# vimalmanohar/old-kaldi-git

Measured on AMD Instinct MI355X. Metric: frames/sec decoded + real-time factor, LibriSpeech nnet2 decode @1/2/4/8 MI355X, higher is better.
Workload: dtype f32

## Files before the change

### old-kaldi-git_amd/csrc/kh_decoder.hip

```cpp
#include <algorithm>
#include <cstddef>
#include <cstdint>

#include "kh_common.h"
#include "kh_decoder_types.h"

using namespace kh;
using namespace kh::dec;

namespace {

__device__ __forceinline__ unsigned KhOpaqueTidX() {
  unsigned t = threadIdx.x;
  asm volatile("" : "+v"(t));
  return t;
}
#define KH_TIDX (KhOpaqueTidX())

#ifdef KH_SERVE_MARKERS
__device__ int32_t *g_serve_mark = nullptr;
#define KM(k, aux) do { if (KH_TIDX == 0 && g_serve_mark != nullptr) __hip_atomic_store(g_serve_mark + blockIdx.x * 16 + 13, ((k) << 24) | (static_cast<int32_t>(aux) & 0xffffff), __ATOMIC_RELAXED, __HIP_MEMORY_SCOPE_SYSTEM); } while (0)
__device__ int32_t *g_wave_mark = nullptr;
#define WM(k, aux) do { if ((KH_TIDX & 63) == 0 && g_wave_mark != nullptr) __hip_atomic_store(g_wave_mark + blockIdx.x * 64 + (KH_TIDX >> 6), ((k) << 24) | (static_cast<int32_t>(aux) & 0xffffff), __ATOMIC_RELAXED, __HIP_MEMORY_SCOPE_SYSTEM); } while (0)
#define WM_ANY(c) (__any(c) ? (1 << 20) : 0)
// ... 1892 lines not shown
      if (cnt != n_new) sh->status = cnt < 0 ? 3 : 8;
    }
  }
  KhSync();
  SubStamp(u, sh, 50);
  if (Uni(sh->status) != 0) return false;
  for (int i = ne_emit + KH_TIDX; i < fe; i += NT)
    __hip_atomic_fetch_min(&UX(x_bmin)[UX(x_bkt)[i - nb]], UX(x_q)[i - nb], __ATOMIC_RELAXED, __HIP_MEMORY_SCOPE_AGENT);
  KhSync();
  {
    constexpr int kOU = 4;
    for (int i0 = KH_TIDX; i0 < n; i0 += NT * kOU) {
      int32_t bk[kOU];
      uint32_t qv[kOU], bm[kOU];
#pragma unroll
      for (int k = 0; k < kOU; k++) {
        const int i = min(i0 + k * NT, n - 1);
        bk[k] = UX(x_bkt)[i];
        qv[k] = UX(x_q)[i];
      }
#pragma unroll
      for (int k = 0; k < kOU; k++) bm[k] = __hip_atomic_load(&UX(x_bmin)[bk[k]], __ATOMIC_RELAXED, __HIP_MEMORY_SCOPE_AGENT);
#pragma unroll
      for (int k = 0; k < kOU; k++) {
        const int i = i0 + k * NT;
        if (i >= n) continue;
        UX(x_key0)[i] = (static_cast<unsigned long long>(bm[k]) << 32) | qv[k];
        UX(x_val0)[i] = i;
      }
    }
  }
  KhSync();
  {
    constexpr int kOU = 4;
    for (int i0 = KH_TIDX; i0 < n; i0 += NT * kOU) {
      int32_t bk[kOU];
#pragma unroll
      for (int k = 0; k < kOU; k++) bk[k] = UX(x_bkt)[min(i0 + k * NT, n - 1)];
#pragma unroll
      for (int k = 0; k < kOU; k++)
        if (i0 + k * NT < n) UX(x_bmin)[bk[k]] = 0xFFFFFFFFu;
    }
  }
  const int fb2 = n > 1 ? BlockRadixSort(u, n, bits, sh) : 0;
  KhSync();
  const Arr<const int32_t> order = fb2 ? UX(x_val1) : UX(x_val0);
  {
    constexpr int kOU = 8;
    for (int r0 = KH_TIDX; r0 < n; r0 += NT * kOU) {
      int32_t o[kOU];
#pragma unroll
      for (int k = 0; k < kOU; k++) o[k] = order[min(r0 + k * NT, n - 1)];
#pragma unroll
      for (int k = 0; k < kOU; k++)
        if (r0 + k * NT < n) UX(x_pos)[o[k]] = r0 + k * NT;
    }
  }
  KhSync();
  SubStamp(u, sh, 51);
  return true;
}

constexpr int kFastN = 65535, kFastNew = 1024, kFastMulti = 2 * kLdsSlots;

__device__ __forceinline__ int OpaqueTid() {
  int t = static_cast<int>(threadIdx.x);
  asm volatile("" : "+v"(t));
  return t;
}
struct TidRef {
  __device__ __forceinline__ operator int() const { return OpaqueTid(); }
};

__device__ __forceinline__ int BitmapPrefix(LdsU32 bits, LdsU32 pre, int W, Blk &sh) {
  const TidRef tid;
  constexpr int kPer = kLdsSlots / NT;
  int c[kPer], mine = 0;
#pragma unroll
  for (int j = 0; j < kPer; j++) {
    const int w = tid * kPer + j;
    const uint32_t v = bits[w];
    c[j] = w < W ? __popc(v) : 0;
    mine += c[j];
  }
  int total;
  int run = BlockExScan<true>(mine, &total, sh);
#pragma unroll
  for (int j = 0; j < kPer; j++) {
    const int w = tid * kPer + j;
    if (w < W) pre[w] = static_cast<uint32_t>(run);
    run += c[j];
  }
  return total;
}
__device__ __forceinline__ int LdsExScanInPlace(LdsU32 a, int W, Blk &sh) {
  const TidRef tid;
  constexpr int kPer = kLdsSlots / NT;
  int c[kPer], mine = 0;
#pragma unroll
  for (int j = 0; j < kPer; j++) {
    const int w = tid * kPer + j;
    const uint32_t v = a[w];
    c[j] = w < W ? static_cast<int>(v) : 0;
    mine += c[j];
  }
  int total;
  int run = BlockExScan<true>(mine, &total, sh);
#pragma unroll
  for (int j = 0; j < kPer; j++) {
    const int w = tid * kPer + j;
    if (w < W) a[w] = static_cast<uint32_t>(run);
    run += c[j];
  }
  return total;
}
__device__ __forceinline__ int BitRank(LdsU32 bits, LdsU32 pre, uint32_t q) {
  return static_cast<int>(pre[q >> 5]) + __popc(bits[q >> 5] & ((1u << (q & 31u)) - 1u));
}

__device__ void ReplayFromMemory(const Utt &u, const Params &p, int nb, int fe, int lb, int le, float cutoff, uint32_t qbase, Blk &sh) {
  const int ne_emit = Uni(sh->x_ne_emit), eps_emit = Uni(sh->x_eps_emit), eps_n = Uni(sh->eps_n), n_new = fe - ne_emit;
  for (int j = KH_TIDX; j < eps_n; j += NT) {
    const int tok = u.tmp_epslist[j];
    UX(x_epsidx)[tok - nb] = j;
    UX(x_nl0)[j] = 0;
    UX(x_nl1)[j] = 0;
    UX(x_ncost)[j] = j < eps_emit ? Dec(UX(x_c0e)[j]) : INFINITY;
  }
  for (int i = ne_emit + KH_TIDX; i < fe; i += NT) UX(x_q)[i - nb] = 0xFFFFFFFFu;
  KhSync();
  for (int l = lb + KH_TIDX; l < le; l += NT) {
    const int src = u.link_src[l], dst = u.link_dst[l];
    const int j = UX(x_epsidx)[src - nb];
    if (l == lb || u.link_src[l - 1] != src) UX(x_nl0)[j] = l - lb;
    if (l + 1 == le || u.link_src[l + 1] != src) UX(x_nl1)[j] = l - lb + 1;
    int code = -1;
    if (dst >= 0) {
      const int e = UX(x_epsidx)[dst - nb];
      if (e >= 0) code = e;
      else if (dst >= ne_emit) code = 0x40000000 | (dst - nb);
    }
    UX(x_ord)[l - lb] = code;
    UX(x_lw)[l - lb] = __int_as_float(p.n_arcs[-1 - u.link_arc[l]].z);
  }
  KhSync();
  if (KH_TIDX == 0) {
    const int cnt = ReplayClosure((GP(float))UX(x_ncost).p, (GP(int32_t))UX(x_nl0).p, (GP(int32_t))UX(x_nl1).p, (GP(int32_t))UX(x_ord).p,
                                  (GP(float))UX(x_lw).p, (GP(int32_t))UX(x_stack).p, 0, u, sh, eps_emit, cutoff, nb, qbase, n_new);
    if (cnt != n_new) sh->status = cnt < 0 ? 3 : 8;
  }
  KhSync();
}

__device__ void PositionsFromHeads(const Utt &u, int cnt, Blk &sh, int xs0) {
  const TidRef tid;
  const LdsU32 K = (LdsU32)LdsKeys(sh);
  constexpr int kU = 8;
  int pbase = 0;
  for (int h0 = 0; h0 < cnt; h0 += kLdsSlots) {
    const uint32_t W = static_cast<uint32_t>(min(kLdsSlots, cnt - h0));
    for (uint32_t w = tid; w < W; w += NT) K[w] = 0u;
    LdsSync();
    XS(xs0 + 0);
    for (int i0 = tid; i0 < cnt; i0 += NT * kU) {
      int hh[kU];
#pragma unroll
      for (int k = 0; k < kU; k++) hh[k] = UX(x_h)[min(i0 + k * NT, cnt - 1)];
#pragma unroll
      for (int k = 0; k < kU; k++) {
        const uint32_t at = static_cast<uint32_t>(hh[k] - h0);
        if (i0 + k * NT < cnt && at < W) (void)__hip_atomic_fetch_add(&K[at], 1u, __ATOMIC_RELAXED, __HIP_MEMORY_SCOPE_WORKGROUP);
      }
    }
    LdsSync();
    XS(xs0 + 1);
    const int total = LdsExScanInPlace(K, static_cast<int>(W), sh);
    LdsSync();
    XS(xs0 + 2);
    for (int i0 = tid; i0 < cnt; i0 += NT * kU) {
      int hh[kU], ib[kU];
#pragma unroll
      for (int k = 0; k < kU; k++) {
        const int i = min(i0 + k * NT, cnt - 1);
        hh[k] = UX(x_h)[i];
        ib[k] = UX(x_inb)[i];
      }
#pragma unroll
      for (int k = 0; k < kU; k++) {
        const uint32_t at = static_cast<uint32_t>(hh[k] - h0);
        if (i0 + k * NT < cnt && at < W) UX(x_pos)[i0 + k * NT] = pbase + static_cast<int>(K[at]) + ib[k];
      }
    }
    pbase += total;
    LdsSync();
    XS(xs0 + 3);
  }
}

__device__ int OrderFrontierFast(const Utt &u, const Params &p, int nb, int fe, int lb, int le, float cutoff, Blk &sh) {
  const TidRef tid;
  const int ne_emit = Uni(sh->x_ne_emit), n = fe - nb, n_emit = ne_emit - nb, eps_emit = Uni(sh->x_eps_emit), eps_n = Uni(sh->eps_n);
  const uint32_t H = Uni(sh->x_hsize), qbase = Uni(sh->x_qbase);
  const int nl = le - lb, n_new = fe - ne_emit;
  const LdsU32 K = (LdsU32)LdsKeys(sh), V = (LdsU32)LdsVals(sh);
  const LdsU16 V16 = (LdsU16)LdsVals(sh);
  const int Hw = static_cast<int>((H + 31u) >> 5), qw = static_cast<int>((qbase + 31u) >> 5);
  const Arr<int32_t> xr = UX(x_val0);
  constexpr int kU = 8;
  if (u.phase_cycles != nullptr && tid == 0) {
    sh->t_sub = static_cast<long long>(__builtin_amdgcn_s_memtime());
    sh->phase[47] += 1; sh->phase[52] += eps_emit; sh->phase[53] += eps_n; sh->phase[54] += nl; sh->phase[55] += n_new; sh->phase[46] += n;
  }
  const bool comb = qw + 2 * Hw <= kLdsSlots;
  const int o1 = comb ? qw : 0, o2 = o1 + Hw, W1 = o2 + Hw;
  if (!comb) {
    int rbase = 0;
    for (uint32_t c0 = 0; c0 < qbase; c0 += static_cast<uint32_t>(kLdsSlots) * 32u) {
      const int W = min(kLdsSlots, static_cast<int>((qbase - c0 + 31u) >> 5));
      for (int w = tid; w < W; w += NT) K[w] = 0u;
      LdsSync();
      XS(0);
      for (int i = tid; i < n_emit; i += NT) {
        const uint32_t q = UX(x_q)[i] - c0;
        if (q < static_cast<uint32_t>(kLdsSlots) * 32u) (void)__hip_atomic_fetch_or(&K[q >> 5], 1u << (q & 31u), __ATOMIC_RELAXED, __HIP_MEMORY_SCOPE_WORKGROUP);
      }
      LdsSync();
      XS(1);
      const int total = BitmapPrefix(K, V, W, sh);
      LdsSync();
      XS(2);
      for (int i = tid; i < n_emit; i += NT) {
        const uint32_t q = UX(x_q)[i] - c0;
        if (q < static_cast<uint32_t>(kLdsSlots) * 32u) xr[i] = rbase + BitRank(K, V, q);
      }
      rbase += total;
      LdsSync();
      XS(3);
    }
  }
  for (int w = tid; w < W1; w += NT) K[w] = 0u;
  LdsSync();
  XS(4);
  for (int i0 = tid; i0 < n; i0 += NT * kU) {
    int32_t sid[kU];
    uint32_t qv[kU];
#pragma unroll
    for (int k = 0; k < kU; k++) {
      const int i = min(i0 + k * NT, n - 1);
      sid[k] = i < n_emit ? UX(x_bkt)[i] : -1 - p.unit_ilabel[u.tok_state[nb + i]];
      qv[k] = UX(x_q)[i];
    }
#pragma unroll
    for (int k = 0; k < kU; k++) {
      const int i = i0 + k * NT;
      if (i >= n) continue;
      const uint32_t bk = static_cast<uint32_t>(sid[k]) % H;
      UX(x_bkt)[i] = static_cast<int32_t>(bk);
      UX(x_epsidx)[i] = -1;
      if (i < n_emit) {
        const uint32_t m = 1u << (bk & 31u);
        const uint32_t old = __hip_atomic_fetch_or(&K[o1 + (bk >> 5)], m, __ATOMIC_RELAXED, __HIP_MEMORY_SCOPE_WORKGROUP);
        if ((old & m) != 0u) (void)__hip_atomic_fetch_or(&K[o2 + (bk >> 5)], m, __ATOMIC_RELAXED, __HIP_MEMORY_SCOPE_WORKGROUP);
        if (comb) (void)__hip_atomic_fetch_or(&K[qv[k] >> 5], 1u << (qv[k] & 31u), __ATOMIC_RELAXED, __HIP_MEMORY_SCOPE_WORKGROUP);
      }
    }
  }
  LdsSync();
  XS(5);
  for (int i = n_emit + static_cast<int>((tid + NT - n_emit % NT) % NT); i < n; i += NT) {
    const uint32_t bk = static_cast<uint32_t>(UX(x_bkt)[i]), m = 1u << (bk & 31u);
    if ((K[o1 + (bk >> 5)] & m) != 0u) (void)__hip_atomic_fetch_or(&K[o2 + (bk >> 5)], m, __ATOMIC_RELAXED, __HIP_MEMORY_SCOPE_WORKGROUP);
  }
  LdsSync();
  XS(6);
  const int n_bits = BitmapPrefix(K, V, W1, sh);
  LdsSync();
  XS(7);
  const int pre2 = static_cast<int>(V[o2]);
  const int n_b2 = n_bits - pre2;
  if (n_b2 > kLdsSlots) return 2;
  for (int i0 = tid; i0 < n; i0 += NT * kU) {
    uint32_t bks[kU], qv[kU];
#pragma unroll
    for (int k = 0; k < kU; k++) {
      const int i = min(i0 + k * NT, n - 1);
      bks[k] = static_cast<uint32_t>(UX(x_bkt)[i]);
      qv[k] = (comb || i >= n_emit) ? UX(x_q)[i] : static_cast<uint32_t>(xr[i]);
    }
#pragma unroll
    for (int k = 0; k < kU; k++) {
      const int i = i0 + k * NT;
      if (i >= n) continue;
      const uint32_t bk = bks[k], m = 1u << (bk & 31u);
      const int w2 = o2 + static_cast<int>(bk >> 5);
      const uint32_t bits2 = K[w2];
      const int r = i < n_emit ? (comb ? BitRank(K, V, qv[k]) : static_cast<int>(qv[k])) : -1;
      if (comb && i < n_emit) xr[i] = r;
      if ((bits2 & m) != 0u) {
        UX(x_bkt)[i] = static_cast<int>(V[w2]) - pre2 + __popc(bits2 & (m - 1u));
      } else {
        UX(x_bkt)[i] = i < n_emit ? -1 : -2 - static_cast<int32_t>(bk);
        UX(x_h)[i] = r;
        UX(x_inb)[i] = 0;
      }
    }
  }
// ... 303 lines not shown
  const int o1 = comb ? qw : 0, o2 = o1 + Hw, W1 = o2 + Hw;
  const LdsU32 P = comb ? K + W1 : K + qw;
  const LdsU32 P2 = comb ? K + W1 + o2 : K + 2 * Hw;
  if (tid == 0) sh->flag = 0;
  if (!comb) {
    for (int w = tid; w < qw; w += NT) K[w] = 0u;
    LdsSync();
    for (int i0 = tid; i0 < n; i0 += NT * kU) {
      int32_t sid[kU];
      uint32_t qv[kU];
#pragma unroll
      for (int k = 0; k < kU; k++) {
        const int i = min(i0 + k * NT, n - 1);
        sid[k] = i < n_emit ? UX(x_bkt)[i] : -1 - p.unit_ilabel[u.tok_state[nb + i]];
        qv[k] = UX(x_q)[i];
      }
#pragma unroll
      for (int k = 0; k < kU; k++) {
        const int i = i0 + k * NT;
        if (i >= n) continue;
        T[i] = static_cast<uint32_t>(sid[k]) % H;
        if (i < n_emit) (void)__hip_atomic_fetch_or(&K[qv[k] >> 5], 1u << (qv[k] & 31u), __ATOMIC_RELAXED, __HIP_MEMORY_SCOPE_WORKGROUP);
      }
    }
    LdsSync();
    (void)BitmapPrefix(K, P, qw, sh);
    LdsSync();
    for (int i = tid; i < n_emit; i += NT) T[i] |= static_cast<uint32_t>(BitRank(K, P, UX(x_q)[i])) << 17;
    LdsSync();
    for (int w = tid; w < 2 * Hw; w += NT) K[w] = 0u;
    LdsSync();
    for (int i = tid; i < n_emit; i += NT) {
      const uint32_t bk = T[i] & 0x1ffffu, m = 1u << (bk & 31u);
      const uint32_t old = __hip_atomic_fetch_or(&K[o1 + (bk >> 5)], m, __ATOMIC_RELAXED, __HIP_MEMORY_SCOPE_WORKGROUP);
      if ((old & m) != 0u) (void)__hip_atomic_fetch_or(&K[o2 + (bk >> 5)], m, __ATOMIC_RELAXED, __HIP_MEMORY_SCOPE_WORKGROUP);
    }
  } else {
    for (int w = tid; w < W1; w += NT) K[w] = 0u;
    LdsSync();
    for (int i0 = tid; i0 < n; i0 += NT * kU) {
      int32_t sid[kU];
      uint32_t qv[kU];
#pragma unroll
      for (int k = 0; k < kU; k++) {
        const int i = min(i0 + k * NT, n - 1);
        sid[k] = i < n_emit ? UX(x_bkt)[i] : -1 - p.unit_ilabel[u.tok_state[nb + i]];
        qv[k] = UX(x_q)[i];
      }
#pragma unroll
      for (int k = 0; k < kU; k++) {
        const int i = i0 + k * NT;
        if (i >= n) continue;
        const uint32_t bk = static_cast<uint32_t>(sid[k]) % H;
        T[i] = bk;
        if (i < n_emit) {
          const uint32_t m = 1u << (bk & 31u);
          const uint32_t old = __hip_atomic_fetch_or(&K[o1 + (bk >> 5)], m, __ATOMIC_RELAXED, __HIP_MEMORY_SCOPE_WORKGROUP);
          if ((old & m) != 0u) (void)__hip_atomic_fetch_or(&K[o2 + (bk >> 5)], m, __ATOMIC_RELAXED, __HIP_MEMORY_SCOPE_WORKGROUP);
          (void)__hip_atomic_fetch_or(&K[qv[k] >> 5], 1u << (qv[k] & 31u), __ATOMIC_RELAXED, __HIP_MEMORY_SCOPE_WORKGROUP);
        }
      }
    }
  }
  LdsSync();
  for (int i = n_emit + tid; i < n; i += NT) {
    const uint32_t bk = T[i] & 0x1ffffu, m = 1u << (bk & 31u);
    if ((K[o1 + (bk >> 5)] & m) != 0u) (void)__hip_atomic_fetch_or(&K[o2 + (bk >> 5)], m, __ATOMIC_RELAXED, __HIP_MEMORY_SCOPE_WORKGROUP);
  }
  LdsSync();
  int n_b2;
  uint32_t pre2 = 0u;
  if (comb) {
    const int n_bits = BitmapPrefix(K, P, W1, sh);
    LdsSync();
    pre2 = Uni(P[o2]);
    n_b2 = n_bits - static_cast<int>(pre2);
  } else {
    n_b2 = BitmapPrefix(K + o2, P2, Hw, sh);
    LdsSync();
  }
  if (n_b2 > kLdsSlots / 2) return 2;
  uint32_t tw[kU];
  int cb[kU];
#pragma unroll
  for (int k = 0; k < kU; k++) {
    tw[k] = 0u;
    cb[k] = -1;
    const int i = tid + k * NT;
    if (i >= n) continue;
    const uint32_t t0 = T[i], bk = t0 & 0x1ffffu, m = 1u << (bk & 31u);
    const uint32_t bits2 = K[o2 + (bk >> 5)];
    uint32_t word = 0u;
    if (i < n_emit) word = comb ? static_cast<uint32_t>(BitRank(K, P, UX(x_q)[i])) : t0 >> 17;
    if ((bits2 & m) != 0u) word |= ((P2[bk >> 5] - pre2 + static_cast<uint32_t>(__popc(bits2 & (m - 1u)))) << 13) | (1u << 26);
    else if (i >= n_emit) cb[k] = static_cast<int>(bk);
    tw[k] = word;
  }
  LdsSync();
  const LdsU32 Cb = K + 7168;
  const LdsU32 Cr = K + 7168 + 512;
#pragma unroll
  for (int k = 0; k < kU; k++) {
    const int i = tid + k * NT;
    if (i >= n) continue;
    T[i] = tw[k];
    if (i >= n_emit) Cb[i - n_emit] = static_cast<uint32_t>(cb[k] + 1);
  }
  const LdsU16 M16 = (LdsU16)(K + kLdsSlots / 2);
  if (n_b2 > 0) {
    for (int w = tid; w < n_b2; w += NT) K[w] = 0u;
    LdsSync();
    for (int i = tid; i < n_emit; i += NT) {
      const uint32_t w = T[i];
      if ((w >> 26) & 1u) (void)__hip_atomic_fetch_add(&K[(w >> 13) & 0x1fffu], 1u, __ATOMIC_RELAXED, __HIP_MEMORY_SCOPE_WORKGROUP);
    }
    LdsSync();
    const int n_multi = LdsExScanInPlace(K, n_b2, sh);
    LdsSync();
    if (n_multi > 2 * (7168 - kLdsSlots / 2)) return 2;
    for (int i = tid; i < n_emit; i += NT) {
      const uint32_t w = T[i];
      if ((w >> 26) & 1u)
        M16[__hip_atomic_fetch_add(&K[(w >> 13) & 0x1fffu], 1u, __ATOMIC_RELAXED, __HIP_MEMORY_SCOPE_WORKGROUP)] = static_cast<uint16_t>(w & 0x1fffu);
    }
    LdsSync();
    bool wide = false;
    for (int i = tid; i < n; i += NT) {
      const uint32_t w = T[i];
      if (((w >> 26) & 1u) == 0u) continue;
      const int d = static_cast<int>((w >> 13) & 0x1fffu);
      const int s0 = d > 0 ? static_cast<int>(K[d - 1]) : 0, s1 = static_cast<int>(K[d]);
      const uint32_t r = i < n_emit ? (w & 0x1fffu) : 0xFFFFFFFFu;
      uint32_t hm = 0xFFFFFFFFu;
      int inb = 0;
      for (int m = s0; m < s1; m++) {
        const uint32_t rr = M16[m];
        hm = rr < hm ? rr : hm;
        inb += rr < r ? 1 : 0;
      }
      wide |= inb > 255;
      T[i] = hm | (static_cast<uint32_t>(inb & 255) << 13);
    }
    if (wide) sh->flag = 1;
  }
  LdsSync();
  if (Uni(sh->flag) != 0) return 2;
  SubStamp(u, sh, 48);
  const LdsU32 kQ = K, kPop = K + 1024;
  const LdsF kNcost = (LdsF)(K + 2048);
  const LdsI kNlr = (LdsI)(K + 3072), kCode = (LdsI)(K + 4096);
  const LdsF kLw = (LdsF)(K + 5120);
  typedef __attribute__((address_space(3))) unsigned long long *LdsU64;
  const LdsU64 key64 = (LdsU64)(K + 6144 + ((reinterpret_cast<uintptr_t>((__attribute__((address_space(3))) void *)(K + 6144)) >> 2) & 1u));
  int my_rank = 0;
  if (n_new > 0) {
    for (int j = tid; j < eps_n; j += NT) {
      const int i = u.tmp_epslist[j] - nb;
      (void)__hip_atomic_fetch_or(&T[i], static_cast<uint32_t>(j + 1) << 21, __ATOMIC_RELAXED, __HIP_MEMORY_SCOPE_WORKGROUP);
      kNcost[j] = j < eps_emit ? Dec(UX(x_c0e)[j]) : INFINITY;
      kNlr[j] = 0;
      if (j < eps_emit) {
        const uint32_t w = T[i];
        kQ[j] = ((w & 0x1fffu) << 8) | ((w >> 13) & 0xffu);
      }
    }
    for (int k = tid; k < n_new; k += NT) key64[k] = ~0ull;
    LdsSync();
    for (int j = tid; j < eps_emit; j += NT) {
      const uint32_t key = kQ[j];
      int rank = 0, j2 = 0;
      for (; j2 + 4 <= eps_emit; j2 += 4) {
        const uint32_t a0 = kQ[j2], a1 = kQ[j2 + 1], a2 = kQ[j2 + 2], a3 = kQ[j2 + 3];
        rank += (a0 < key ? 1 : 0) + (a1 < key ? 1 : 0) + (a2 < key ? 1 : 0) + (a3 < key ? 1 : 0);
      }
      for (; j2 < eps_emit; j2++) rank += kQ[j2] < key ? 1 : 0;
      kPop[j] = static_cast<uint32_t>(eps_emit - 1 - rank);
    }
    {
      constexpr int kLU = 4;
      for (int l0 = lb + tid; l0 < le; l0 += NT * kLU) {
        int srcs[kLU], dsts[kLU], arcs[kLU], prevs[kLU], nexts[kLU];
        float ws[kLU];
#pragma unroll
        for (int k = 0; k < kLU; k++) {
          const int l = min(l0 + k * NT, le - 1);
          srcs[k] = u.link_src[l];
          dsts[k] = u.link_dst[l];
          arcs[k] = u.link_arc[l];
          prevs[k] = l > lb ? u.link_src[l - 1] : -1;
          nexts[k] = l + 1 < le ? u.link_src[l + 1] : -1;
        }
#pragma unroll
        for (int k = 0; k < kLU; k++) ws[k] = __int_as_float(p.n_arcs[-1 - arcs[k]].z);
#pragma unroll
        for (int k = 0; k < kLU; k++) {
          const int l = l0 + k * NT;
          if (l >= le) continue;
          const int js = static_cast<int>(T[srcs[k] - nb] >> 21) - 1;
          int rng = 0;
          if (prevs[k] != srcs[k]) rng |= l - lb;
          if (nexts[k] != srcs[k]) rng |= (l - lb + 1) << 16;
          if (rng != 0) (void)__hip_atomic_fetch_or(&kNlr[js], rng, __ATOMIC_RELAXED, __HIP_MEMORY_SCOPE_WORKGROUP);
          int code = -1;
          if (dsts[k] >= 0) {
            const int e = static_cast<int>(T[dsts[k] - nb] >> 21) - 1;
            if (e >= 0) code = e | ((dsts[k] >= ne_emit ? dsts[k] - ne_emit + 1 : 0) << 12);
            else if (dsts[k] >= ne_emit) code = 0x40000000 | (dsts[k] - ne_emit);
          }
          kCode[l - lb] = code;
          kLw[l - lb] = ws[k];
        }
      }
    }
    LdsSync();
    for (int j = tid; j < eps_emit; j += NT) {
      const float c0 = kNcost[j];
      if (c0 > cutoff) continue;
      const unsigned long long pop = static_cast<unsigned long long>(kPop[j]) << 40;
      const int r = kNlr[j];
      for (int l = r & 0xffff; l < (r >> 16); l++) {
        int code = kCode[l];
        if (code < 0) continue;
        float tot = c0 + kLw[l];
        if (!(tot < cutoff)) continue;
        for (unsigned long long depth = 1;; depth++) {
          const bool leaf = (code & 0x40000000) != 0;
          const int k = leaf ? (code & 0x3fffffff) : (code >> 12) - 1;
          if (k < 0 || depth > 30) { sh->flag = 1; break; }
          (void)__hip_atomic_fetch_min(&key64[k], pop | (depth << 32) | static_cast<unsigned long long>(l), __ATOMIC_RELAXED, __HIP_MEMORY_SCOPE_WORKGROUP);
          if (leaf) break;
          const int r2 = kNlr[code & 0xfff];
          int l2 = -1;
          for (int ll = r2 & 0xffff; ll < (r2 >> 16); ll++)
            if (kCode[ll] >= 0) { if (l2 >= 0) sh->flag = 1; l2 = ll; }
          if (l2 < 0) break;
          tot = tot + kLw[l2];
          if (!(tot < cutoff)) break;
          code = kCode[l2];
        }
      }
    }
    LdsSync();
    bool bad = false;
    if (tid < n_new) {
      const unsigned long long mine = key64[tid];
      bad = mine == ~0ull;
      const unsigned long long my_pop = mine >> 40, my_depth = (mine >> 32) & 0xffull, my_chain = mine & 0xffffffffull;
      for (int k2 = 0; k2 < n_new; k2++) {
        const unsigned long long o = key64[k2];
        my_rank += o < mine ? 1 : 0;
        if (k2 != tid && (o >> 40) == my_pop) {
          const unsigned long long od = (o >> 32) & 0xffull;
          if (od == my_depth && (my_depth >= 2 || o == mine)) bad = true;
          if (my_depth >= 2 && od >= 2 && (o & 0xffffffffull) != my_chain) bad = true;
        }
      }
    }
    if (bad) sh->flag = 1;
    LdsSync();
    if (Uni(sh->flag) != 0) return 2;
    if (u.phase_cycles != nullptr && tid == 0) sh->phase[64] += 1;
    if (tid < n_new) Cr[tid] = static_cast<uint32_t>(n_emit + my_rank);
    LdsSync();
    if (tid < n_new) {
      const int i = n_emit + tid;
      const uint32_t w = T[i], r = Cr[tid], alone = Cb[tid];
      const uint32_t key = alone != 0u ? alone : 0x80000000u | (w & 0x1fffu);
      uint32_t minr = r;
      int before = 0;
      for (int k2 = 0; k2 < n_new; k2++) {
        const uint32_t a2 = Cb[k2];
        const uint32_t key2 = a2 != 0u ? a2 : 0x80000000u | (T[n_emit + k2] & 0x1fffu);
        if (key2 != key) continue;
        const uint32_t r2 = Cr[k2];
        before += r2 < r ? 1 : 0;
        minr = r2 < minr ? r2 : minr;
      }
      const int inb = (alone != 0u ? 0 : static_cast<int>((w >> 13) & 0xffu)) + before;
      if (inb > 255) sh->flag = 1;
      my_rank = static_cast<int>((alone != 0u ? minr : (w & 0x1fffu)) | (static_cast<uint32_t>(inb & 255) << 13));
    }
    LdsSync();
    if (Uni(sh->flag) != 0) return 2;
    if (tid < n_new) T[n_emit + tid] = (T[n_emit + tid] & 0xffe00000u) | static_cast<uint32_t>(my_rank);
  }
  SubStamp(u, sh, 50);
  for (int w = tid; w < n; w += NT) K[w] = 0u;
  LdsSync();
  for (int i = tid; i < n; i += NT) (void)__hip_atomic_fetch_add(&K[T[i] & 0x1fffu], 1u, __ATOMIC_RELAXED, __HIP_MEMORY_SCOPE_WORKGROUP);
  LdsSync();
  (void)LdsExScanInPlace(K, n, sh);
  LdsSync();
  for (int i = tid; i < n; i += NT) {
    const uint32_t w = T[i];
    UX(x_pos)[i] = static_cast<int>(K[w & 0x1fffu]) + static_cast<int>((w >> 13) & 0xffu);
  }
  KhSync();
  SubStamp(u, sh, 51);
  if (u.phase_cycles != nullptr && tid == 0) {
    sh->phase[47] += 1; sh->phase[52] += eps_emit; sh->phase[53] += eps_n; sh->phase[54] += nl; sh->phase[55] += n_new; sh->phase[46] += n;
    sh->phase[66] += 1;
  }
  return 1;
}

__device__ bool OrderFrontier(const Utt &u, const Params &p, int nb, int fe, int lb, int le, float cutoff, Blk &sh) {
  const int n = fe - nb, n_new = fe - Uni(sh->x_ne_emit);
  const uint32_t H = Uni(sh->x_hsize);
  const bool fast = p.exact_order == 1 && n >= 1 && n <= kFastN && 2u * ((H + 31u) >> 5) <= static_cast<uint32_t>(kLdsSlots) && n_new <= kFastNew &&
                    Uni(sh->x_qbase) < 0x7fffffffu;
  long long t0 = 0;
  if (u.phase_cycles != nullptr && KH_TIDX == 0) {
    t0 = static_cast<long long>(__builtin_amdgcn_s_memtime());
    sh->phase[n <= 8160 ? 61 : (n <= 16384 ? 62 : 63)] += 1;
  }
  int rc = 2;
  if (fast) rc = OrderFrontierLds(u, p, nb, fe, lb, le, cutoff, sh);
  if (fast && rc == 2) rc = OrderFrontierFast(u, p, nb, fe, lb, le, cutoff, sh);
  if (u.phase_cycles != nullptr && KH_TIDX == 0) {
    const long long t1 = static_cast<long long>(__builtin_amdgcn_s_memtime());
    if (rc == 1) sh->phase[59] += t1 - t0;
    t0 = t1;
  }
  if (rc == 2) {
    rc = OrderFrontierSort(u, p, nb, fe, lb, le, cutoff, sh) ? 1 : 0;
    if (u.phase_cycles != nullptr && KH_TIDX == 0) {
      sh->phase[60] += static_cast<long long>(__builtin_amdgcn_s_memtime()) - t0;
      sh->phase[57] += 1;
    }
  }
  return rc == 1;
}

__device__ bool ProcessEmittingExact(const Utt &u, const Params &p, int frame, int b, int e, float *next_cutoff_out, int *cand_out,
                                     Blk &sh) {
  const int nb = Uni(sh->tok_end);
  const int tok_limit = min(u.tok_cap, nb + u.tok_frame_cap);
  const int n = e - b;
  if (KH_TIDX == 0) { sh->wl_n[0] = 0; sh->wl_n[1] = 0; sh->eps_n = 0; sh->erel_n = 0; }
  XS(27);
  StageScoreRow(u, p, sh, frame);
  Stamp(u, sh, 15);
  XS(24);
  const Cutoff c = GetCutoff<true>(u, p, b, e, sh);
  Stamp(u, sh, 0);
  XS(25);
  const int link_frame_b = Uni(sh->link_end);
  if (KH_TIDX == 0) {
    if (c.count > sh->max_tokens_frame) sh->max_tokens_frame = c.count;
    const uint32_t new_sz = static_cast<uint32_t>(static_cast<float>(c.count) * p.hash_ratio);
    if (new_sz > sh->x_hsize) sh->x_hsize = new_sz;
  }
  const float inf = INFINITY;
  float cost_offset = 0.0f;
  float est = inf;
  if (c.best_tok >= 0) {
    cost_offset = -c.best_cost;
    const int32_t s = u.tok_state[c.best_tok];
    const float tot = c.best_cost;
    const int ab = s + 1, ae = ab + p.rec[s].x;
    for (int a = ab + KH_TIDX; a < ae; a += NT) {
      const KhInt4 arc = p.rec[a];
      const float w = __int_as_float(arc.z) + (cost_offset - LogLike(u, p, sh, frame, arc.x));
      const float new_weight = w + tot;
      est = fminf(est, new_weight + c.adaptive_beam);
    }
  }
  if (KH_TIDX == 0) {
    u.cost_offset[frame] = cost_offset;
    sh->work_cursor = b;
    sh->link_cursor = link_frame_b;
  }
  Arr<const KhInt4> x_rec = p.rec;
  Arr<uint32_t> x_cost = u.tok_cost;
  Arr<int32_t> x_state = u.tok_state;
  GP(const float) x_ll = u.ll + static_cast<size_t>(frame) * u.ll_stride;
  int x_ll_cols = p.ll_cols;
  Arr<int32_t> xp_pos = UX(x_pos), xp_c = UX(x_c), xp_ord = UX(x_ord), xp_csid = UX(x_csid);
  Arr<uint32_t> xp_m = UX(x_m);
  Arr<int32_t> x_dst = u.link_dst, x_src = u.link_src, x_arc = u.link_arc;
  Arr<float> x_k = u.link_k, x_a = u.link_a;
  int x_keep_ac = p.keep_ac;
  LaunderOne(x_rec.p); LaunderOne(x_cost.p); LaunderOne(x_state.p); LaunderOne(x_ll); LaunderOne(x_ll_cols);
  LaunderOne(xp_pos.p); LaunderOne(xp_c.p); LaunderOne(xp_m.p); LaunderOne(xp_ord.p); LaunderOne(xp_csid.p);
  LaunderOne(x_dst.p); LaunderOne(x_src.p); LaunderOne(x_arc.p); LaunderOne(x_k.p); LaunderOne(x_a.p);
  LaunderOne(x_keep_ac);
  OwnerScan os = OwnerScanInit(sh);
  const float est0 = BlockMinF(est, sh);
  XS(59);
  constexpr int kCB = 16;
  if (KH_TIDX < kCB) sh->x_cb[KH_TIDX] = Enc(est0);
  const int bshift = n > kCB ? 32 - __clz(n - 1) - 4 : 0;
  const int limit = min(u.link_cap, link_frame_b + u.link_frame_cap);
  constexpr int kScanLds = kLdsSlots - kLdsSlots / 32;
  const bool lds_scan = n <= kScanLds;
  constexpr int kMidBits = 2 * kLdsSlots / 32, kMidBitBase = kLdsSlots - kMidBits;
  const bool mid_scan = !lds_scan && n <= 2 * kLdsSlots && x_ll_cols <= kMidBitBase && p.max_emit < 65536 && p.exact_order == 1;
  const bool key_ord = (lds_scan || mid_scan) && p.max_emit < 65536;
  const LdsU32 sK = (LdsU32)LdsKeys(sh);
  const LdsU32 sV = (LdsU32)LdsVals(sh);
  if (lds_scan)
    for (int w = n + static_cast<int>(KH_TIDX); w < n + ((n + 31) >> 5); w += NT) sK[w] = 0u;
  if (mid_scan) {
    for (int w = KH_TIDX; w < kMidBits; w += NT) sV[kMidBitBase + w] = 0u;
    if (KH_TIDX == 0) sh->x_nbp = 0;
  }
  LdsSync();
  const int lane = KH_TIDX & 63;
  long long my_arcs = 0;
  auto seg_min_scan = [&](float m, int lo) -> float {
#define KH_SEG_STEP(ctrl, rm) { const float nm = __int_as_float(DppMov<ctrl, rm>(0x7f800000, __float_as_int(m))); const int nlo = DppMov<ctrl, rm>(-2, lo); if (nlo == lo) m = fminf(m, nm); }
    KH_SEG_STEP(0x111, 0xf) KH_SEG_STEP(0x112, 0xf) KH_SEG_STEP(0x114, 0xf) KH_SEG_STEP(0x118, 0xf) KH_SEG_STEP(0x142, 0xa) KH_SEG_STEP(0x143, 0xc)
#undef KH_SEG_STEP
    return m;
  };
  int base_next = WaveLdsFetchAdd(&sh->work_cursor, 64);
  uint32_t co_next = 0u;
  int st_next = 0, pos_next = 0;
  if (base_next < e) {
    const int icn = min(base_next + lane, e - 1);
    co_next = LoadCostEnc(&x_cost[icn]);
    st_next = x_state[icn];
    pos_next = xp_pos[icn - b];
  }
  for (;;) {
    const int base = base_next;
    if (base >= e) break;
    const int i = base + lane;
    const bool in_range = i < e;
    const uint32_t co = co_next;
    int st = st_next;
    const int pos = pos_next;
    const int blk = pos >> bshift;
    base_next = WaveLdsFetchAdd(&sh->work_cursor, 64);
    if (base_next < e) {
      const int icn = min(base_next + lane, e - 1);
      co_next = LoadCostEnc(&x_cost[icn]);
// ... 2220 lines not shown
```

Measured before the change: 1.543 million.

## Split rank/closure scans across lane groups with shuffle reductions in epsilon ordering

The O(n^2) rank computations for queue tokens and closure tokens previously used one thread per token, leaving most of the block idle when counts are small. They now split each token's scan across a power-of-two group of lanes and combine partial counts and minima with wavefront shuffles. Link metadata is loaded into registers once per lane, and the arc-weight gather is issued before the rank pass to overlap its latency. This relies on static bounds that put links and tokens within one block, and adds shuffle overhead plus extra XS markers.

```diff
diff --git a/old-kaldi-git_amd/csrc/kh_decoder.hip b/old-kaldi-git_amd/csrc/kh_decoder.hip
--- a/old-kaldi-git_amd/csrc/kh_decoder.hip
+++ b/old-kaldi-git_amd/csrc/kh_decoder.hip
@@ -2068,6 +2068,34 @@
   KhSync();
 }
 
+__device__ __forceinline__ int PairLanesLog2(int n) {
+  int lg = 0;
+  while (lg < 6 && (n << (lg + 1)) <= NT) lg++;
+  return lg;
+}
+__device__ __forceinline__ int GroupSumI(int v, int lg, int lane) {
+  for (int m = 1; m < (1 << lg); m <<= 1) v += ShflI(v, lane ^ m);
+  return v;
+}
+__device__ __forceinline__ uint32_t GroupMinU(uint32_t v, int lg, int lane) {
+  for (int m = 1; m < (1 << lg); m <<= 1) {
+    const uint32_t o = static_cast<uint32_t>(ShflI(static_cast<int>(v), lane ^ m));
+    v = o < v ? o : v;
+  }
+  return v;
+}
+__device__ __forceinline__ int RankBelow(LdsU32 keys, int n, int lg, int t, uint32_t key) {
+  const int n4 = (n + 3) & ~3;
+  const int chunk = (((n4 >> 2) + (1 << lg) - 1) >> lg) << 2;
+  const int a = (t & ((1 << lg) - 1)) * chunk, b = min(a + chunk, n4);
+  int rank = 0;
+  for (int j2 = a; j2 < b; j2 += 4) {
+    const uint32_t a0 = keys[j2], a1 = keys[j2 + 1], a2 = keys[j2 + 2], a3 = keys[j2 + 3];
+    rank += (a0 < key ? 1 : 0) + (a1 < key ? 1 : 0) + (a2 < key ? 1 : 0) + (a3 < key ? 1 : 0);
+  }
+  return GroupSumI(rank, lg, t & 63);
+}
+
 __device__ void PositionsFromHeads(const Utt &u, int cnt, Blk &sh, int xs0) {
   const TidRef tid;
   const LdsU32 K = (LdsU32)LdsKeys(sh);
@@ -2677,8 +2705,18 @@
   const LdsF kLw = (LdsF)(K + 5120);
   typedef __attribute__((address_space(3))) unsigned long long *LdsU64;
   const LdsU64 key64 = (LdsU64)(K + 6144 + ((reinterpret_cast<uintptr_t>((__attribute__((address_space(3))) void *)(K + 6144)) >> 2) & 1u));
+  static_assert(kT1Links <= NT && kT1Nodes <= NT && 2 * kT1New <= NT, "a lane per link, a lane group per queue token / closure token");
   int my_rank = 0;
   if (n_new > 0) {
+    int l_src = 0, l_dst = -1, l_arc = 0, l_prev = -1, l_next = -1;
+    if (tid < nl) {
+      const int l = lb + tid;
+      l_src = u.link_src[l];
+      l_dst = u.link_dst[l];
+      l_arc = u.link_arc[l];
+      l_prev = tid > 0 ? u.link_src[l - 1] : -1;
+      l_next = tid + 1 < nl ? u.link_src[l + 1] : -1;
+    }
     for (int j = tid; j < eps_n; j += NT) {
       const int i = u.tmp_epslist[j] - nb;
       (void)__hip_atomic_fetch_or(&T[i], static_cast<uint32_t>(j + 1) << 21, __ATOMIC_RELAXED, __HIP_MEMORY_SCOPE_WORKGROUP);
@@ -2690,54 +2728,34 @@
       }
     }
     for (int k = tid; k < n_new; k += NT) key64[k] = ~0ull;
+    if (tid < 3 && eps_emit + tid < ((eps_emit + 3) & ~3)) kQ[eps_emit + tid] = 0xFFFFFFFFu;
     LdsSync();
-    for (int j = tid; j < eps_emit; j += NT) {
-      const uint32_t key = kQ[j];
-      int rank = 0, j2 = 0;
-      for (; j2 + 4 <= eps_emit; j2 += 4) {
-        const uint32_t a0 = kQ[j2], a1 = kQ[j2 + 1], a2 = kQ[j2 + 2], a3 = kQ[j2 + 3];
-        rank += (a0 < key ? 1 : 0) + (a1 < key ? 1 : 0) + (a2 < key ? 1 : 0) + (a3 < key ? 1 : 0);
-      }
-      for (; j2 < eps_emit; j2++) rank += kQ[j2] < key ? 1 : 0;
-      kPop[j] = static_cast<uint32_t>(eps_emit - 1 - rank);
-    }
+    XS(50);
+    float l_w = 0.0f;
+    if (tid < nl) l_w = __int_as_float(p.n_arcs[-1 - l_arc].z);
     {
-      constexpr int kLU = 4;
-      for (int l0 = lb + tid; l0 < le; l0 += NT * kLU) {
-        int srcs[kLU], dsts[kLU], arcs[kLU], prevs[kLU], nexts[kLU];
-        float ws[kLU];
-#pragma unroll
-        for (int k = 0; k < kLU; k++) {
-          const int l = min(l0 + k * NT, le - 1);
-          srcs[k] = u.link_src[l];
-          dsts[k] = u.link_dst[l];
-          arcs[k] = u.link_arc[l];
-          prevs[k] = l > lb ? u.link_src[l - 1] : -1;
-          nexts[k] = l + 1 < le ? u.link_src[l + 1] : -1;
-        }
-#pragma unroll
-        for (int k = 0; k < kLU; k++) ws[k] = __int_as_float(p.n_arcs[-1 - arcs[k]].z);
-#pragma unroll
-        for (int k = 0; k < kLU; k++) {
-          const int l = l0 + k * NT;
-          if (l >= le) continue;
-          const int js = static_cast<int>(T[srcs[k] - nb] >> 21) - 1;
-          int rng = 0;
-          if (prevs[k] != srcs[k]) rng |= l - lb;
-          if (nexts[k] != srcs[k]) rng |= (l - lb + 1) << 16;
-          if (rng != 0) (void)__hip_atomic_fetch_or(&kNlr[js], rng, __ATOMIC_RELAXED, __HIP_MEMORY_SCOPE_WORKGROUP);
-          int code = -1;
-          if (dsts[k] >= 0) {
-            const int e = static_cast<int>(T[dsts[k] - nb] >> 21) - 1;
-            if (e >= 0) code = e | ((dsts[k] >= ne_emit ? dsts[k] - ne_emit + 1 : 0) << 12);
-            else if (dsts[k] >= ne_emit) code = 0x40000000 | (dsts[k] - ne_emit);
-          }
-          kCode[l - lb] = code;
-          kLw[l - lb] = ws[k];
-        }
-      }
+      const int lg = PairLanesLog2(eps_emit), j = tid >> lg;
+      const int rank = RankBelow(kQ, eps_emit, lg, tid, j < eps_emit ? kQ[j] : 0u);
+      if (j < eps_emit && (tid & ((1 << lg) - 1)) == 0) kPop[j] = static_cast<uint32_t>(eps_emit - 1 - rank);
+    }
+    XS(51);
+    if (tid < nl) {
+      const int js = static_cast<int>(T[l_src - nb] >> 21) - 1;
+      int rng = 0;
+      if (l_prev != l_src) rng |= tid;
+      if (l_next != l_src) rng |= (tid + 1) << 16;
+      if (rng != 0) (void)__hip_atomic_fetch_or(&kNlr[js], rng, __ATOMIC_RELAXED, __HIP_MEMORY_SCOPE_WORKGROUP);
+      int code = -1;
+      if (l_dst >= 0) {
+        const int e = static_cast<int>(T[l_dst - nb] >> 21) - 1;
+        if (e >= 0) code = e | ((l_dst >= ne_emit ? l_dst - ne_emit + 1 : 0) << 12);
+        else if (l_dst >= ne_emit) code = 0x40000000 | (l_dst - ne_emit);
+      }
+      kCode[tid] = code;
+      kLw[tid] = l_w;
     }
     LdsSync();
+    XS(52);
     for (int j = tid; j < eps_emit; j += NT) {
       const float c0 = kNcost[j];
       if (c0 > cutoff) continue;
@@ -2766,34 +2784,40 @@
       }
     }
     LdsSync();
+    XS(53);
+    const int lg7 = PairLanesLog2(n_new), L7 = 1 << lg7, ck = tid >> lg7, cs = tid & (L7 - 1);
+    const bool c_on = ck < n_new;
     bool bad = false;
-    if (tid < n_new) {
-      const unsigned long long mine = key64[tid];
+    if (c_on) {
+      const unsigned long long mine = key64[ck];
       bad = mine == ~0ull;
       const unsigned long long my_pop = mine >> 40, my_depth = (mine >> 32) & 0xffull, my_chain = mine & 0xffffffffull;
-      for (int k2 = 0; k2 < n_new; k2++) {
+      for (int k2 = cs; k2 < n_new; k2 += L7) {
         const unsigned long long o = key64[k2];
         my_rank += o < mine ? 1 : 0;
-        if (k2 != tid && (o >> 40) == my_pop) {
+        if (k2 != ck && (o >> 40) == my_pop) {
           const unsigned long long od = (o >> 32) & 0xffull;
           if (od == my_depth && (my_depth >= 2 || o == mine)) bad = true;
           if (my_depth >= 2 && od >= 2 && (o & 0xffffffffull) != my_chain) bad = true;
         }
       }
     }
+    my_rank = GroupSumI(my_rank, lg7, tid & 63);
     if (bad) sh->flag = 1;
     LdsSync();
     if (Uni(sh->flag) != 0) return 2;
+    XS(54);
     if (u.phase_cycles != nullptr && tid == 0) sh->phase[64] += 1;
-    if (tid < n_new) Cr[tid] = static_cast<uint32_t>(n_emit + my_rank);
+    if (c_on && cs == 0) Cr[ck] = static_cast<uint32_t>(n_emit + my_rank);
     LdsSync();
-    if (tid < n_new) {
-      const int i = n_emit + tid;
-      const uint32_t w = T[i], r = Cr[tid], alone = Cb[tid];
+    uint32_t w = 0u, alone = 0u, minr = 0xFFFFFFFFu;
+    int before = 0;
+    if (c_on) {
+      w = T[n_emit + ck];
+      alone = Cb[ck];
+      const uint32_t r = Cr[ck];
       const uint32_t key = alone != 0u ? alone : 0x80000000u | (w & 0x1fffu);
-      uint32_t minr = r;
-      int before = 0;
-      for (int k2 = 0; k2 < n_new; k2++) {
+      for (int k2 = cs; k2 < n_new; k2 += L7) {
         const uint32_t a2 = Cb[k2];
         const uint32_t key2 = a2 != 0u ? a2 : 0x80000000u | (T[n_emit + k2] & 0x1fffu);
         if (key2 != key) continue;
@@ -2801,13 +2825,18 @@
         before += r2 < r ? 1 : 0;
         minr = r2 < minr ? r2 : minr;
       }
+    }
+    before = GroupSumI(before, lg7, tid & 63);
+    minr = GroupMinU(minr, lg7, tid & 63);
+    if (c_on && cs == 0) {
       const int inb = (alone != 0u ? 0 : static_cast<int>((w >> 13) & 0xffu)) + before;
       if (inb > 255) sh->flag = 1;
       my_rank = static_cast<int>((alone != 0u ? minr : (w & 0x1fffu)) | (static_cast<uint32_t>(inb & 255) << 13));
     }
     LdsSync();
     if (Uni(sh->flag) != 0) return 2;
-    if (tid < n_new) T[n_emit + tid] = (T[n_emit + tid] & 0xffe00000u) | static_cast<uint32_t>(my_rank);
+    if (c_on && cs == 0) T[n_emit + ck] = (w & 0xffe00000u) | static_cast<uint32_t>(my_rank);
+    XS(55);
   }
   SubStamp(u, sh, 50);
   for (int w = tid; w < n; w += NT) K[w] = 0u;
```

Result: no change. 1.550 million (median of 6 runs) (+0.5%).
